# NIRVANALAN/CVPR23-E3DGE

Measured on AMD Instinct MI355X. Metric: rendered_rays_per_sec_64x64x24, higher is better.
Workload: dtype f32 (operands split f16 hi+lo, 3 f16 MFMA products, fp32 accumulate)

## Files before the change

cvpr23-e3dge_amd/csrc/siren16.h:

```cpp
#pragma once
#include "siren_common.h"

namespace e3dge {

typedef float f32x4v __attribute__((ext_vector_type(4)));

constexpr int k16Threads = 512;
constexpr int k16Tiles = 16;
constexpr int k16Steps = 8;
constexpr int k16ChunkFloats = 16 * kWidth;
constexpr int k16Chunks = kBigLayers * k16Tiles;
#ifndef E3DGE_16_ABL
#define E3DGE_16_ABL 0
#endif
constexpr int k16NBuf = 4;
constexpr int k16Slots = 2;
#ifndef E3DGE_16_RING
#define E3DGE_16_RING 2
#endif
constexpr int k16Ring = E3DGE_16_RING;

constexpr int k16LdsW = 0;
constexpr int k16LdsFilm = k16LdsW + k16NBuf * k16ChunkFloats;
constexpr int k16LdsHead = k16LdsFilm + 9 * 2 * kWidth;
constexpr int k16LdsW0 = k16LdsHead + kHeadFloats;
constexpr int k16LdsWvt = k16LdsW0 + 3 * kWidth;
constexpr int k16LdsFeat = k16LdsWvt + 3 * kWidth;
constexpr int k16LdsPart = k16LdsFeat + kRMax * kFPitch;
constexpr int k16LdsAlpha = ((k16LdsPart + 8 * k16Slots * kWidth + 3) / 4) * 4;
constexpr int k16LdsWgt = k16LdsAlpha + kTilePts;
constexpr int k16LdsZ = k16LdsWgt + kTilePts;
constexpr int k16LdsPts = k16LdsZ + kTilePts;
constexpr int k16LdsRgb = k16LdsPts + kTilePts * 3;
constexpr int k16LdsState = k16LdsRgb + kTilePts * 3;
constexpr int k16LdsWq = ((k16LdsState + kRMax * kStateStride + 3) / 4) * 4;
constexpr int k16LdsVd = k16LdsWq + 8 * k16Slots * 16;
constexpr int k16LdsFloats = k16LdsVd + 8 * 16 * 4;
constexpr int k16LdsBytes = k16LdsFloats * 4;
static_assert(k16LdsBytes <= 160 * 1024, "LDS budget");
static_assert((k16LdsFilm % 4) == 0 && (k16LdsHead % 4) == 0 && (k16LdsW0 % 4) == 0 && (k16LdsWvt % 4) == 0, "alignment");

#ifndef E3DGE_NT_STORES
#define E3DGE_NT_STORES 1
#endif
__device__ __forceinline__ void save_st4(float* p, const f32x4v& v) {
#if E3DGE_NT_STORES
    __builtin_nontemporal_store(v, reinterpret_cast<f32x4v*>(p));
#else
    *reinterpret_cast<f32x4v*>(p) = v;
#endif
}
__device__ __forceinline__ f32x4v mfma16x16(u32x4 a, u32x4 b, f32x4v c) {
    return __builtin_amdgcn_mfma_f32_16x16x32_f16(__builtin_bit_cast(half8, a), __builtin_bit_cast(half8, b), c, 0, 0, 0);
}
__device__ __forceinline__ f32x4v zero4() { return f32x4v{0.f, 0.f, 0.f, 0.f}; }
template <int HI> __device__ __forceinline__ float fma_mix_h(unsigned p, float w, float acc) {
    float r;
    if (HI) asm("v_fma_mix_f32 %0, %1, %2, %3 op_sel:[1,0,0] op_sel_hi:[1,0,0]" : "=v"(r) : "v"(p), "v"(w), "v"(acc));
    else asm("v_fma_mix_f32 %0, %1, %2, %3 op_sel:[0,0,0] op_sel_hi:[1,0,0]" : "=v"(r) : "v"(p), "v"(w), "v"(acc));
    return r;
}
__device__ __forceinline__ float act16_get(const u32x4 (&aH)[k16Steps], const u32x4 (&aL)[k16Steps], int t, int r) {
    const int g = t >> 1, w = 2 * (t & 1) + (r >> 1);
    return (r & 1) ? f16hi(aH[g][w]) + f16hi(aL[g][w]) : f16lo(aH[g][w]) + f16lo(aL[g][w]);
}
template <int CTRL> __device__ __forceinline__ float dpp16(float x) {
    return __builtin_bit_cast(float, __builtin_amdgcn_update_dpp(0, __builtin_bit_cast(int, x), CTRL, 0xf, 0xf, true));
}
__device__ __forceinline__ float row_sum16(float x) {
    x += dpp16<0x128>(x);
    x += dpp16<0x124>(x);
    x += dpp16<0x122>(x);
    x += dpp16<0x121>(x);
    return x;
}

__device__ __forceinline__ float sum_over_q(float x) {
    const unsigned u = __builtin_bit_cast(unsigned, x);
    const auto r = __builtin_amdgcn_permlane16_swap(u, u, false, false);
    const float y = __builtin_bit_cast(float, (unsigned)r[0]) + __builtin_bit_cast(float, (unsigned)r[1]);
    const unsigned v = __builtin_bit_cast(unsigned, y);
    const auto t = __builtin_amdgcn_permlane32_swap(v, v, false, false);
    return __builtin_bit_cast(float, (unsigned)t[0]) + __builtin_bit_cast(float, (unsigned)t[1]);
}

template <int CTRL, int ROW_MASK> __device__ __forceinline__ float dpp_or(float ident, float x) {
    return __builtin_bit_cast(float, __builtin_amdgcn_update_dpp(__builtin_bit_cast(int, ident), __builtin_bit_cast(int, x), CTRL, ROW_MASK, 0xf, false));
}
__device__ __forceinline__ float wave_incl_prod(float x) {
    x = __fmul_rn(x, dpp_or<0x111, 0xf>(1.0f, x));
    x = __fmul_rn(x, dpp_or<0x112, 0xf>(1.0f, x));
    x = __fmul_rn(x, dpp_or<0x114, 0xf>(1.0f, x));
    x = __fmul_rn(x, dpp_or<0x118, 0xf>(1.0f, x));
    x = __fmul_rn(x, dpp_or<0x142, 0xa>(1.0f, x));
    x = __fmul_rn(x, dpp_or<0x143, 0xc>(1.0f, x));
    return x;
}
__device__ __forceinline__ float wave_sum_last(float x) {
    x = __fadd_rn(x, dpp_or<0x111, 0xf>(0.0f, x));
    x = __fadd_rn(x, dpp_or<0x112, 0xf>(0.0f, x));
    x = __fadd_rn(x, dpp_or<0x114, 0xf>(0.0f, x));
    x = __fadd_rn(x, dpp_or<0x118, 0xf>(0.0f, x));
    x = __fadd_rn(x, dpp_or<0x142, 0xa>(0.0f, x));
    x = __fadd_rn(x, dpp_or<0x143, 0xc>(0.0f, x));
    return __builtin_bit_cast(float, __builtin_amdgcn_readlane(__builtin_bit_cast(int, x), 63));
}

struct ChunkPipe16 {
    const char* img;
    uint32_t voff, lds_base;
    int idx, buf, use_buf, count;
    float* wbuf;
    const float* wcur;
    const float* wnxt;
    __device__ __forceinline__ void init(float* wbuf_, const float* image, int wave, int lane, int count_ = k16Chunks) {
        const int wave_u = __builtin_amdgcn_readfirstlane(wave);
        wbuf = wbuf_;
        count = count_;
        img = reinterpret_cast<const char*>(image) + wave_u * 2048;
        voff = (uint32_t)lane * 16u;
        lds_base = (uint32_t)(size_t)(__attribute__((address_space(3))) float*)wbuf_ + (uint32_t)wave_u * 2048u;
        idx = 0; buf = 0; use_buf = 0;
        wcur = wbuf_; wnxt = wbuf_ + k16ChunkFloats;
    }
    __device__ __forceinline__ void issue_chunk() {
        const char* s = img + (size_t)idx * (k16ChunkFloats * 4);
        const uint32_t d = lds_base + (uint32_t)buf * (k16ChunkFloats * 4);
        glds16_saddr<0>(s, voff, d);
        glds16_saddr<1024>(s, voff, d);
        idx = (idx + 1 == count) ? 0 : idx + 1;
        buf = (buf + 1 == k16NBuf) ? 0 : buf + 1;
    }
    __device__ __forceinline__ void prime() {
        issue_chunk(); issue_chunk(); issue_chunk();
    }
#ifdef E3DGE_PHASE_TIMING
    unsigned long long t_vm = 0, t_bar = 0;
#endif
    template <bool STRICT> __device__ __forceinline__ void sync() {
#ifdef E3DGE_PHASE_TIMING
        const unsigned long long c0 = __builtin_readcyclecounter();
#endif
        if (STRICT) asm volatile("s_waitcnt vmcnt(0)" ::: "memory");
        else asm volatile("s_waitcnt vmcnt(2)" ::: "memory");
#ifdef E3DGE_PHASE_TIMING
        const unsigned long long c1 = __builtin_readcyclecounter();
#endif
#if !(E3DGE_16_ABL & 4)
        __syncthreads();
#endif
#ifdef E3DGE_PHASE_TIMING
        t_vm += c1 - c0; t_bar += __builtin_readcyclecounter() - c1;
#endif
    }
    __device__ __forceinline__ void advance() {
        use_buf = (use_buf + 1 == k16NBuf) ? 0 : use_buf + 1;
        wcur = wnxt;
        wnxt = wbuf + ((use_buf + 1 == k16NBuf) ? 0 : use_buf + 1) * k16ChunkFloats;
    }
};

#ifdef E3DGE_16_TRACE
__device__ unsigned long long g_trace16[2][24];
#define TRACE16_STAMP(i) do { if (trace) asm volatile("s_memtime %0" : "=s"(tstamp[i])); } while (0)
#else
#define TRACE16_STAMP(i) do { } while (0)
#endif

template <bool TRANSPOSED, int RING = k16Ring, class Epi, class Hook>
__device__ __forceinline__ void tile16(ChunkPipe16& pipe, int lane, const u32x4 (&aH)[k16Steps], const u32x4 (&aL)[k16Steps],
                                       f32x4v& acc, f32x4v& accb, u32x4 (&ringH)[RING], u32x4 (&ringL)[RING], Epi&& epi,
                                       Hook&& hook, int sbuf = -1, [[maybe_unused]] int trace = 0) {
#ifdef E3DGE_16_TRACE
    unsigned long long tstamp[24];
#endif
    const u32x4* __restrict__ wp = reinterpret_cast<const u32x4*>(sbuf >= 0 ? pipe.wbuf + sbuf * k16ChunkFloats : pipe.wcur) + lane;
    const u32x4* __restrict__ wn = reinterpret_cast<const u32x4*>(sbuf >= 0 ? pipe.wbuf + ((sbuf + 1) % k16NBuf) * k16ChunkFloats : pipe.wnxt) + lane;
#pragma unroll
    for (int g = 0; g < k16Steps; ++g) {
        const int ga = g + RING - 1;
        TRACE16_STAMP(3 * g);
        ringH[ga % RING] = (ga < k16Steps) ? wp[(ga * 2 + 0) * 64] : wn[((ga - k16Steps) * 2 + 0) * 64];
        ringL[ga % RING] = (ga < k16Steps) ? wp[(ga * 2 + 1) * 64] : wn[((ga - k16Steps) * 2 + 1) * 64];
        __builtin_amdgcn_sched_barrier(0);
        const u32x4 wh = ringH[g % RING], wl = ringL[g % RING];
        f32x4v& x0 = (g & 1) ? accb : acc;
        f32x4v& x1 = (g & 1) ? acc : accb;
        if (!TRANSPOSED) {
            x0 = mfma16x16(wh, aH[g], x0);
            x1 = mfma16x16(wl, aH[g], x1);
            x0 = mfma16x16(wh, aL[g], x0);
        } else {
            x0 = mfma16x16(aH[g], wh, x0);
            x1 = mfma16x16(aH[g], wl, x1);
            x0 = mfma16x16(aL[g], wh, x0);
        }
        TRACE16_STAMP(3 * g + 1);
        if (g == 1) hook();
        epi(g);
        TRACE16_STAMP(3 * g + 2);
    }
#ifdef E3DGE_16_TRACE
    if (trace) {
        asm volatile("s_waitcnt lgkmcnt(0)" ::: "memory");
        if ((threadIdx.x & 63) == 0)
            for (int i = 0; i < 24; ++i) g_trace16[trace - 1][i] = tstamp[i];
    }
#endif
}

#ifndef E3DGE_16_HELPERS_ONLY
#ifdef E3DGE_PHASE_TIMING
#define PHASE16(i) do { if (MODE == 0 && blockIdx.x == 0 && tid == 0 && sub < 3) tstamp[sub * 6 + (i)] = __builtin_readcyclecounter(); } while (0)
#else
#define PHASE16(i) do { } while (0)
#endif

constexpr int64_t k16SlabWords = 8 * 2 * 64;

template <int MODE, bool SAVE, int CACHE = 0>
__global__ void __launch_bounds__(k16Threads) siren16_kernel(const SirenK a) {
    static_assert(CACHE == 0 || (MODE == 0 && !SAVE), "the backbone hand-over exists for inference renders only");
    extern __shared__ __attribute__((aligned(16))) float smem[];
    float* const wbuf = smem + k16LdsW;
    float* const film_s = smem + k16LdsFilm;
    float* const head_s = smem + k16LdsHead;
    float* const w0_s = smem + k16LdsW0;
    float* const wvt_s = smem + k16LdsWvt;
    float* const feat_acc = smem + k16LdsFeat;
    float* const part = smem + k16LdsPart;
    float* const alpha_s = smem + k16LdsAlpha;
    float* const wgt_s = smem + k16LdsWgt;
    float* const z_s = smem + k16LdsZ;
    float* const pts_s = smem + k16LdsPts;
    float* const rgb_s = smem + k16LdsRgb;
    float* const state = smem + k16LdsState;

    const int tid_k = threadIdx.x;
#ifdef E3DGE_PHASE_TIMING
    const unsigned long long t_entry = __builtin_readcyclecounter();
    unsigned long long t_loop0 = 0, t_loop1 = 0;
#endif
    int b, npts, n_sub;
    int pix0 = 0, nrays = 0;
    long long pt0 = 0;
    const int S = (MODE == 0) ? a.S : 1;
    if (MODE == 0) {
        b = blockIdx.x / a.tiles_per_img;
        const int tile = blockIdx.x - b * a.tiles_per_img;
        const int HW = a.H * a.Wd;
        pix0 = tile * a.R;
        nrays = min(a.R, HW - pix0);
        npts = nrays * S;
    } else {
        b = blockIdx.x / a.wgs_per_img;
        const int wg = blockIdx.x - b * a.wgs_per_img;
        pt0 = (long long)wg * a.subtiles_per_wg * kTilePts;
        const long long rem = a.n_pts - pt0;
        npts = (int)(rem < (long long)a.subtiles_per_wg * kTilePts ? rem : (long long)a.subtiles_per_wg * kTilePts);
    }
    n_sub = (npts + kTilePts - 1) / kTilePts;

    const float* __restrict__ packed = a.packed;
    const float* __restrict__ film_g = a.film + (int64_t)b * 9 * 2 * kWidth;
    ChunkPipe16 pipe;
    if (CACHE == 2) pipe.init(wbuf, packed + kOffBig16b + (int64_t)(kBigLayers - 1) * k16Tiles * k16ChunkFloats, tid_k >> 6, tid_k & 63, k16Tiles);
    else pipe.init(wbuf, packed + kOffBig16b, tid_k >> 6, tid_k & 63);
    pipe.prime();
    for (int i = tid_k; i < 9 * kWidth; i += k16Threads) {
        const int l = i >> 8, n = i & 255;
        const float gm = film_g[(l * 2 + 0) * kWidth + n], bt = film_g[(l * 2 + 1) * kWidth + n];
        film_s[(l * 2 + 0) * kWidth + n] = (l >= 1) ? gm * (1.0f / kW16Scale) : gm;
        film_s[(l * 2 + 1) * kWidth + n] = __fadd_rn(__fmul_rn(gm, packed[kOffBias + l * kWidth + n]), bt);
    }
    for (int i = tid_k; i < kHeadFloats; i += k16Threads) head_s[i] = packed[kOffWSigma + i];
    for (int i = tid_k; i < 3 * kWidth; i += k16Threads) {
        const int c = i >> 8, n = i & 255;
        const int src = ((n >> 5) * 2 + (c >> 1)) * 64 + (c & 1) * 32 + (n & 31);
        w0_s[i] = packed[kOffFirst + src];
        wvt_s[i] = packed[kOffVTail + src] * kW16Scale;
    }
    float cw[12] = {0}, focal = 1.f, nearv = 0.f, farv = 0.f;
    if (MODE == 0) {
#pragma unroll
        for (int i = 0; i < 12; ++i) cw[i] = a.c2w[b * 12 + i];
        focal = a.focal[b]; nearv = a.near[b]; farv = a.far[b];
        for (int i = tid_k; i < kRMax * kStateStride; i += k16Threads) state[i] = 0.0f;
        for (int i = tid_k; i < kRMax * kFPitch; i += k16Threads) feat_acc[i] = 0.0f;
    }
    const float* __restrict__ film = film_s;

    asm volatile("s_waitcnt vmcnt(0)" ::: "memory");
    __syncthreads();
    u32x4 ringH[k16Ring], ringL[k16Ring];
    {
        const int lane0 = tid_k & 63;
#pragma unroll
        for (int g = 0; g < k16Ring - 1; ++g) {
            ringH[g] = reinterpret_cast<const u32x4*>(pipe.wcur)[(g * 2 + 0) * 64 + lane0];
            ringL[g] = reinterpret_cast<const u32x4*>(pipe.wcur)[(g * 2 + 1) * 64 + lane0];
        }
    }

#ifdef E3DGE_16_TRACE
    auto trace_sel = [&](int L, int t) {
        const int w = __builtin_amdgcn_readfirstlane(tid_k >> 6);
        return (MODE == 0 && blockIdx.x == 7 && L == 3 && t == 6 && (w == 0 || w == 4)) ? 1 + (w >> 2) : 0;
    };
#else
    auto trace_sel = [](int, int) { return 0; };
#endif
    auto fwd_hook = [&](int younger) {
        if (SAVE) {
            switch (younger) {
                case 2: asm volatile("s_waitcnt vmcnt(2)" ::: "memory"); break;
                case 3: asm volatile("s_waitcnt vmcnt(3)" ::: "memory"); break;
                default: asm volatile("s_waitcnt vmcnt(4)" ::: "memory"); break;
            }
            asm volatile("s_waitcnt lgkmcnt(0)\n\ts_barrier" ::: "memory");
        } else {
            pipe.template sync<false>();
        }
        pipe.issue_chunk();
    };
    u32x4 inH[k16Steps], inL[k16Steps], outH[k16Steps], outL[k16Steps];
#ifdef E3DGE_PHASE_TIMING
    unsigned long long tstamp[18];
    for (int i = 0; i < 18; ++i) tstamp[i] = 0;
#endif

#ifdef E3DGE_PHASE_TIMING
    t_loop0 = __builtin_readcyclecounter();
#endif
    for (int sub = 0; sub < n_sub; ++sub) {
        int tid_o = tid_k;
        asm volatile("" : "+v"(tid_o));
        const int tid = tid_o, lane = tid & 63, wave = tid >> 6, q = lane >> 4, col = lane & 15;
        PHASE16(0);
        const int p_sub = 16 * wave + col;
        const int p = sub * kTilePts + p_sub;
        const bool valid = p < npts;
        const int pc = valid ? p : (npts - 1);
        float px = 0.f, py = 0.f, pz = 0.f, vx = 0.f, vy = 0.f, vz = 0.f, zval = 0.f, dist = 0.f;
        int ray_l = 0, s_idx = 0;
        int64_t gpt;
        if (MODE == 0) {
            ray_l = pc / S;
            s_idx = pc - ray_l * S;
            const int pix = pix0 + ray_l;
            const int iy = pix / a.Wd, ix = pix - iy * a.Wd;
            gpt = ((int64_t)b * a.H * a.Wd + pix) * S + s_idx;
            const float hres = (float)a.res * 0.5f;
            const float d0 = __fdiv_rn(((float)ix + 0.5f) - hres, focal);
            const float d1 = -__fdiv_rn(((float)iy + 0.5f) - hres, focal);
            const float d2 = -1.0f;
            float rd[3];
#pragma unroll
            for (int m = 0; m < 3; ++m)
                rd[m] = __fadd_rn(__fadd_rn(__fmul_rn(d0, cw[4 * m + 0]), __fmul_rn(d1, cw[4 * m + 1])), __fmul_rn(d2, cw[4 * m + 2]));
            const float dn = sqrtf(__fadd_rn(__fadd_rn(__fmul_rn(d0, d0), __fmul_rn(d1, d1)), __fmul_rn(d2, d2)));
            vx = __fdiv_rn(d0, dn); vy = __fdiv_rn(d1, dn); vz = __fdiv_rn(d2, dn);
            const float tv = a.t_vals[s_idx];
            zval = __fadd_rn(__fmul_rn(nearv, __fsub_rn(1.0f, tv)), __fmul_rn(farv, tv));
            px = __fadd_rn(cw[3], __fmul_rn(rd[0], zval));
            py = __fadd_rn(cw[7], __fmul_rn(rd[1], zval));
            pz = __fadd_rn(cw[11], __fmul_rn(rd[2], zval));
            const float rdn = sqrtf(__fadd_rn(__fadd_rn(__fmul_rn(rd[0], rd[0]), __fmul_rn(rd[1], rd[1])), __fmul_rn(rd[2], rd[2])));
            if (s_idx + 1 < S) {
                const float tn = a.t_vals[s_idx + 1];
                const float zn = __fadd_rn(__fmul_rn(nearv, __fsub_rn(1.0f, tn)), __fmul_rn(farv, tn));
                dist = __fmul_rn(__fsub_rn(zn, zval), rdn);
            } else {
                dist = __fmul_rn(1e10f, rdn);
            }
            if (valid && q == 0) {
                if (a.points) { float* o = a.points + gpt * 3; o[0] = px; o[1] = py; o[2] = pz; }
                if (a.dists) a.dists[gpt] = dist;
                if (s_idx == 0) {
                    const int64_t gr = (int64_t)b * a.H * a.Wd + pix;
                    if (a.rays_d) { float* o = a.rays_d + gr * 3; o[0] = rd[0]; o[1] = rd[1]; o[2] = rd[2]; }
                    if (a.viewdirs) { float* o = a.viewdirs + gr * 3; o[0] = vx; o[1] = vy; o[2] = vz; }
                }
            }
        } else {
            gpt = (int64_t)b * a.n_pts + pt0 + pc;
            const float* pp = a.pts + gpt * 3;
            px = pp[0]; py = pp[1]; pz = pp[2];
            if (a.vdirs) { const float* vv = a.vdirs + gpt * 3; vx = vv[0]; vy = vv[1]; vz = vv[2]; }
        }
        const int64_t gpt_block = (MODE == 0) ? ((int64_t)b * a.H * a.Wd + pix0) * S : (int64_t)b * a.n_pts + pt0;
        const bool sblk = SAVE && a.save_blocked != 0;
        const int64_t img_n = (MODE == 0) ? (int64_t)a.H * a.Wd * S : (int64_t)a.n_pts;
        const int64_t srow_block = (int64_t)b * saved_rows_per_image(sblk, img_n) + ((MODE == 0) ? (int64_t)pix0 * S : pt0);
        float* const sv = SAVE ? a.save_args + saved_row_floats(sblk, srow_block + pc, q, 9) : nullptr;
        const int sv_ls = sblk ? kSlabLayerF : kWidth, sv_ts = sblk ? kSlabTileF : 16;
        float* const vd_s = smem + k16LdsVd + wave * 64;
        if (q == 0) { vd_s[col * 4 + 0] = vx; vd_s[col * 4 + 1] = vy; vd_s[col * 4 + 2] = vz; }

        if (CACHE != 2) {
            const float xs = __fmul_rn(px, a.box_scale), ys = __fmul_rn(py, a.box_scale), zs = __fmul_rn(pz, a.box_scale);
#pragma unroll
            for (int t = 0; t < k16Tiles; ++t) {
                const int o = 16 * t + 4 * q;
                const f32x4v wx = *reinterpret_cast<const f32x4v*>(w0_s + o), wy = *reinterpret_cast<const f32x4v*>(w0_s + kWidth + o),
                             wz = *reinterpret_cast<const f32x4v*>(w0_s + 2 * kWidth + o);
                const f32x4v g4 = *reinterpret_cast<const f32x4v*>(film + o), b4 = *reinterpret_cast<const f32x4v*>(film + kWidth + o);
                f32x4v arg, v;
#pragma unroll
                for (int r = 0; r < 4; ++r) {
                    const float lin = fmaf(wz[r], zs, fmaf(wy[r], ys, wx[r] * xs));
                    arg[r] = fmaf(g4[r], lin, b4[r]);
                    v[r] = sin_f32(arg[r]);
                }
                if (SAVE) save_st4(sv + t * sv_ts, arg);
                SPLIT2_TO(v[0], v[1], inH[t >> 1][2 * (t & 1)], inL[t >> 1][2 * (t & 1)]);
                SPLIT2_TO(v[2], v[3], inH[t >> 1][2 * (t & 1) + 1], inL[t >> 1][2 * (t & 1) + 1]);
            }
        }

        PHASE16(1);
#pragma unroll 1
        for (int L = 1; L < ((CACHE == 2) ? 0 : E3DGE_SIREN_DEPTH); ++L) {
            const float* __restrict__ film_l = film + L * 2 * kWidth;
            f32x4v prev = zero4();
            auto finish = [&](int tp, const f32x4v& pv) {
                const int o = 16 * tp + 4 * q;
                const f32x4v g4 = *reinterpret_cast<const f32x4v*>(film_l + o), b4 = *reinterpret_cast<const f32x4v*>(film_l + kWidth + o);
                f32x4v arg, v;
#pragma unroll
                for (int r = 0; r < 4; ++r) { arg[r] = fmaf(g4[r], pv[r], b4[r]); v[r] = sin_f32(arg[r]); }
                if (SAVE) save_st4(sv + L * sv_ls + tp * sv_ts, arg);
                SPLIT2_TO(v[0], v[1], outH[tp >> 1][2 * (tp & 1)], outL[tp >> 1][2 * (tp & 1)]);
                SPLIT2_TO(v[2], v[3], outH[tp >> 1][2 * (tp & 1) + 1], outL[tp >> 1][2 * (tp & 1) + 1]);
            };
#pragma unroll
            for (int t = 0; t < k16Tiles; ++t) {
                f32x4v acc = zero4(), accb = zero4();
                if (t == 0) {
                    tile16<false>(pipe, lane, inH, inL, acc, accb, ringH, ringL, [](int) {}, [&]() { fwd_hook(2); }, t % k16NBuf);
                } else {
                    const int o = 16 * (t - 1) + 4 * q;
                    f32x4v g4 = zero4(), b4 = zero4(), arg4 = zero4(), kf4 = zero4(), x4 = zero4();
                    tile16<false>(pipe, lane, inH, inL, acc, accb, ringH, ringL, [&](int g) {
                        if (g == 0) {
                            g4 = *reinterpret_cast<const f32x4v*>(film_l + o);
                            b4 = *reinterpret_cast<const f32x4v*>(film_l + kWidth + o);
                        } else if (g == 1) {
#pragma unroll
                            for (int r = 0; r < 4; ++r) arg4[r] = fmaf(g4[r], prev[r], b4[r]);
#ifndef E3DGE_POLY_SINE
#pragma unroll
                            for (int r = 0; r < 4; ++r) kf4[r] = rintf(arg4[r] * 0.15915494f);
                        } else if (g == 2) {
#pragma unroll
                            for (int r = 0; r < 4; ++r) kf4[r] = fmaf(arg4[r], 6.4206382e-09f, fmaf(arg4[r], 0.15915494f, -kf4[r]));
#endif
                        } else if (g == 3) {
#pragma unroll
#ifndef E3DGE_POLY_SINE
                            for (int r = 0; r < 4; ++r) x4[r] = __builtin_amdgcn_sinf(kf4[r]);
#else
                            for (int r = 0; r < 4; ++r) x4[r] = sin_poly_f32(arg4[r]);
#endif
                            if (SAVE) save_st4(sv + L * sv_ls + (t - 1) * sv_ts, arg4);
                        } else if (g == 4) {
                            SPLIT2_TO(x4[0], x4[1], outH[(t - 1) >> 1][2 * ((t - 1) & 1)], outL[(t - 1) >> 1][2 * ((t - 1) & 1)]);
                            SPLIT2_TO(x4[2], x4[3], outH[(t - 1) >> 1][2 * ((t - 1) & 1) + 1], outL[(t - 1) >> 1][2 * ((t - 1) & 1) + 1]);
                        }
                    }, [&]() { fwd_hook(t < 2 ? 2 : (t == 2 ? 3 : 4)); }, t % k16NBuf, trace_sel(L, t));
                }
                pipe.advance();
                prev = acc + accb;
            }
            finish(k16Tiles - 1, prev);
#pragma unroll
            for (int g = 0; g < k16Steps; ++g) { inH[g] = outH[g]; inL[g] = outL[g]; }
        }

        if (CACHE != 0) {
            const int64_t rec = (((int64_t)blockIdx.x * a.bb_subs + sub) * 8 + wave) * k16SlabWords + lane;
            if (CACHE == 1) {
                u32x4* __restrict__ dst = reinterpret_cast<u32x4*>(a.bb_out) + rec;
#pragma unroll
                for (int g = 0; g < k16Steps; ++g) { dst[(g * 2 + 0) * 64] = inH[g]; dst[(g * 2 + 1) * 64] = inL[g]; }
            } else {
                const u32x4* __restrict__ src = reinterpret_cast<const u32x4*>(a.bb_in) + rec;
#pragma unroll
                for (int g = 0; g < k16Steps; ++g) { inH[g] = src[(g * 2 + 0) * 64]; inL[g] = src[(g * 2 + 1) * 64]; }
            }
        }

        PHASE16(2);
        float sdf = 0.0f;
        if (CACHE == 2) {
            if (q == 0) wgt_s[p_sub] = valid ? a.weights_in[gpt] : 0.0f;
        } else {
            float acc = 0.0f;
#pragma unroll
            for (int t = 0; t < k16Tiles; ++t) {
                const f32x4v w4 = *reinterpret_cast<const f32x4v*>(head_s + 16 * t + 4 * q);
                const int g = t >> 1, w0i = 2 * (t & 1);
                acc = fma_mix_h<0>(inH[g][w0i], w4[0], acc); acc = fma_mix_h<0>(inL[g][w0i], w4[0], acc);
                acc = fma_mix_h<1>(inH[g][w0i], w4[1], acc); acc = fma_mix_h<1>(inL[g][w0i], w4[1], acc);
                acc = fma_mix_h<0>(inH[g][w0i + 1], w4[2], acc); acc = fma_mix_h<0>(inL[g][w0i + 1], w4[2], acc);
                acc = fma_mix_h<1>(inH[g][w0i + 1], w4[3], acc); acc = fma_mix_h<1>(inL[g][w0i + 1], w4[3], acc);
            }
            sdf = sum_over_q(acc) + head_s[4 * kWidth];
        }

        if (MODE == 0 && CACHE != 2) {
            const float sg = __fdiv_rn(sigmoid_f32(__fdiv_rn(-sdf, a.sigmoid_beta)), a.sigmoid_beta);
            const float alpha = __fsub_rn(1.0f, expf(-__fmul_rn(sg, dist)));
            if (q == 0) {
                alpha_s[p_sub] = valid ? alpha : 0.0f;
                z_s[p_sub] = zval;
                pts_s[p_sub * 3 + 0] = px; pts_s[p_sub * 3 + 1] = py; pts_s[p_sub * 3 + 2] = pz;
                if (valid && a.sdf) a.sdf[gpt] = sdf;
            }
            __syncthreads();
            const int sub_lo = sub * kTilePts;
            const int sub_hi = min(sub_lo + kTilePts, npts);
            const int r_first = sub_lo / S, r_last = (sub_hi - 1) / S;
            for (int i = __builtin_amdgcn_readfirstlane(wave); i <= ((E3DGE_16_ABL & 8) ? -1 : r_last - r_first); i += 8) {
                const int rl = r_first + i;
                const int s_lo = max(0, sub_lo - rl * S), s_hi = min(S, sub_hi - rl * S);
                float* st = state + rl * kStateStride;
                float T_in = (s_lo == 0) ? 1.0f : st[0];
                float wsum = (s_lo == 0) ? 0.0f : st[1];
                float dep = 0.0f, x0 = 0.0f, x1 = 0.0f, x2 = 0.0f;
                for (int c0 = s_lo; c0 < s_hi; c0 += 64) {
                    const int s = c0 + lane;
                    const bool act = s < s_hi;
                    const int ps = rl * S + min(s, s_hi - 1) - sub_lo;
                    const float al = act ? alpha_s[ps] : 0.0f;
                    const float zz = z_s[ps], p0 = pts_s[ps * 3 + 0], p1 = pts_s[ps * 3 + 1], p2 = pts_s[ps * 3 + 2];
                    const float incl = wave_incl_prod(act ? __fadd_rn(__fsub_rn(1.0f, al), 1e-10f) : 1.0f);
                    const float T = __fmul_rn(T_in, dpp_or<0x138, 0xf>(1.0f, incl));
                    float w = __fmul_rn(al, T);
                    const bool last = a.force_bg && act && s == S - 1;
                    const float wfront = wave_sum_last(last ? 0.0f : w);
                    if (last) w = __fsub_rn(1.0f, __fadd_rn(wsum, wfront));
                    wsum = __fadd_rn(wsum, wfront);
                    if (act) wgt_s[ps] = w;
                    dep = __fadd_rn(dep, wave_sum_last(__fmul_rn(w, zz)));
                    x0 = __fadd_rn(x0, wave_sum_last(__fmul_rn(w, p0)));
                    x1 = __fadd_rn(x1, wave_sum_last(__fmul_rn(w, p1)));
                    x2 = __fadd_rn(x2, wave_sum_last(__fmul_rn(w, p2)));
                    T_in = __fmul_rn(T_in, __builtin_bit_cast(float, __builtin_amdgcn_readlane(__builtin_bit_cast(int, incl), 63)));
                }
                if (lane == 0) {
                    st[0] = T_in; st[1] = wsum;
                    st[2] = __fadd_rn(st[2], dep); st[3] = __fadd_rn(st[3], x0); st[4] = __fadd_rn(st[4], x1); st[5] = __fadd_rn(st[5], x2);
                }
            }
            __syncthreads();
            if (valid && q == 0 && a.weights) a.weights[gpt] = wgt_s[p_sub];
        }

        if (MODE == 0 && a.tex_alpha) {
            const float* __restrict__ ta = a.tex_alpha + gpt * kWidth;
            const float* __restrict__ tb = a.tex_beta + gpt * kWidth;
#pragma unroll
            for (int t = 0; t < k16Tiles; ++t) {
                const f32x4v a4 = *reinterpret_cast<const f32x4v*>(ta + 16 * t + 4 * q);
                const f32x4v b4 = *reinterpret_cast<const f32x4v*>(tb + 16 * t + 4 * q);
                float y[4];
#pragma unroll
                for (int r = 0; r < 4; ++r) y[r] = __fadd_rn(__fmul_rn(__fadd_rn(a4[r], 1.0f), act16_get(inH, inL, t, r)), b4[r]);
                SPLIT2_TO(y[0], y[1], inH[t >> 1][2 * (t & 1)], inL[t >> 1][2 * (t & 1)]);
                SPLIT2_TO(y[2], y[3], inH[t >> 1][2 * (t & 1) + 1], inL[t >> 1][2 * (t & 1) + 1]);
            }
        }

        PHASE16(3);
        float* const wq_s = smem + k16LdsWq + wave * (k16Slots * 16);
        int slab_first_ray = 0, slab_nslots = 0;
        const int slab_p0 = sub * kTilePts + 16 * wave;
        if (MODE == 0) {
            const int slab_hi = min(slab_p0 + 16, npts);
            if (slab_hi > slab_p0) {
                slab_first_ray = slab_p0 / S;
                slab_nslots = (slab_hi - 1) / S - slab_first_ray + 1;
            }
            const int b1 = (slab_first_ray + 1) * S - slab_p0;
            if (lane < 16) {
                const float w = (slab_p0 + lane < npts) ? wgt_s[16 * wave + lane] : 0.0f;
                wq_s[lane] = (lane < b1) ? w : 0.0f;
                wq_s[16 + lane] = (lane >= b1) ? w : 0.0f;
            }
        }
        const f32x4v q0 = (MODE == 0) ? *reinterpret_cast<const f32x4v*>(wq_s + 4 * q) : zero4();
        const f32x4v q1 = (MODE == 0) ? *reinterpret_cast<const f32x4v*>(wq_s + 16 + 4 * q) : zero4();
        float dvx[4], dvy[4], dvz[4];
#pragma unroll
        for (int r = 0; r < 4; ++r) { dvx[r] = vd_s[(4 * q + r) * 4 + 0]; dvy[r] = vd_s[(4 * q + r) * 4 + 1]; dvz[r] = vd_s[(4 * q + r) * 4 + 2]; }
        float prgb[3][4];
#pragma unroll
        for (int c = 0; c < 3; ++c)
#pragma unroll
            for (int r = 0; r < 4; ++r) prgb[c][r] = 0.0f;
        {
            const float* __restrict__ film_v = film + 8 * 2 * kWidth;
            const float* __restrict__ wrgb = head_s + kWidth;
            f32x4v pv = zero4();
            float e_gm = 0.f, e_bt = 0.f, e_w0 = 0.f, e_w1 = 0.f, e_w2 = 0.f, fa0 = 0.f, fa1 = 0.f;
            int e_n = 0;
            auto epi_begin = [&](int tp) {
                e_n = 16 * tp + col;
                e_gm = film_v[e_n]; e_bt = film_v[kWidth + e_n];
                e_w0 = wrgb[e_n]; e_w1 = wrgb[kWidth + e_n]; e_w2 = wrgb[2 * kWidth + e_n];
                fa0 = fa1 = 0.f;
            };
            auto epi_r = [&](int r) {
                const float varg = fmaf(e_gm, pv[r], e_bt);
                const float h = sin_f32(varg);
                const int pr = slab_p0 + 4 * q + r;
                if (SAVE && pr < npts) a.save_args[saved_elem_floats(sblk, srow_block + pr, 8, e_n, 9)] = varg;
                prgb[0][r] = fmaf(e_w0, h, prgb[0][r]);
                prgb[1][r] = fmaf(e_w1, h, prgb[1][r]);
                prgb[2][r] = fmaf(e_w2, h, prgb[2][r]);
                if (MODE == 0) {
                    fa0 = fmaf(q0[r], h, fa0);
                    fa1 = fmaf(q1[r], h, fa1);
                } else if (a.raw) {
                    if (pr < npts) a.raw[((int64_t)b * a.n_pts + pt0 + pr) * 260 + 4 + e_n] = h;
                }
            };
            auto epi_end = [&]() {
                if (MODE == 0) {
                    fa0 = sum_over_q(fa0);
                    fa1 = sum_over_q(fa1);
                    if (q == 0) {
                        float* pp = part + (wave * k16Slots) * kWidth + e_n;
                        if (slab_nslots > 0) pp[0] = fa0;
                        if (slab_nslots > 1) pp[kWidth] = fa1;
                    }
                }
            };
#pragma unroll 1
            for (int t = 0; t < k16Tiles; ++t) {
                f32x4v acc = zero4(), accb = zero4();
                if (t == 0) {
                    tile16<true>(pipe, lane, inH, inL, acc, accb, ringH, ringL, [](int) {}, [&]() { fwd_hook(2); });
                } else {
                    epi_begin(t - 1);
                    tile16<true>(pipe, lane, inH, inL, acc, accb, ringH, ringL, [&](int g) { if (g >= 1 && g <= 4) epi_r(g - 1); }, [&]() { fwd_hook(2); });
                    epi_end();
                }
                pipe.advance();
                acc = acc + accb;
                const int n = 16 * t + col;
                const float t0 = wvt_s[n], t1 = wvt_s[kWidth + n], t2 = wvt_s[2 * kWidth + n];
#pragma unroll
                for (int r = 0; r < 4; ++r) acc[r] = fmaf(t2, dvz[r], fmaf(t1, dvy[r], fmaf(t0, dvx[r], acc[r])));
                pv = acc;
            }
            epi_begin(k16Tiles - 1);
#pragma unroll
            for (int r = 0; r < 4; ++r) epi_r(r);
            epi_end();
        }

        PHASE16(4);
        float rgbv[3][4];
#pragma unroll
        for (int c = 0; c < 3; ++c)
#pragma unroll
            for (int r = 0; r < 4; ++r) rgbv[c][r] = row_sum16(prgb[c][r]) + head_s[4 * kWidth + 1 + c];
        if (MODE == 0) {
            if (col == 0) {
#pragma unroll
                for (int r = 0; r < 4; ++r) {
                    const int ps = 16 * wave + 4 * q + r;
                    rgb_s[ps * 3 + 0] = sigmoid_f32(rgbv[0][r]);
                    rgb_s[ps * 3 + 1] = sigmoid_f32(rgbv[1][r]);
                    rgb_s[ps * 3 + 2] = sigmoid_f32(rgbv[2][r]);
                }
            }
            __syncthreads();
            const int sub_lo = sub * kTilePts;
            const int sub_hi = min(sub_lo + kTilePts, npts);
            const int r_first = sub_lo / S, r_last = (sub_hi - 1) / S;
            for (int i = __builtin_amdgcn_readfirstlane(wave); i <= ((E3DGE_16_ABL & 16) ? -1 : r_last - r_first); i += 8) {
                const int rl = r_first + i;
                const int s_lo = max(0, sub_lo - rl * S), s_hi = min(S, sub_hi - rl * S);
                float c0 = 0.0f, c1 = 0.0f, c2 = 0.0f;
                for (int b0 = s_lo; b0 < s_hi; b0 += 64) {
                    const int s = b0 + lane;
                    const int ps = rl * S + min(s, s_hi - 1) - sub_lo;
                    const float ww = (s < s_hi) ? wgt_s[ps] : 0.0f;
                    c0 = __fadd_rn(c0, wave_sum_last(__fmul_rn(ww, rgb_s[ps * 3 + 0])));
                    c1 = __fadd_rn(c1, wave_sum_last(__fmul_rn(ww, rgb_s[ps * 3 + 1])));
                    c2 = __fadd_rn(c2, wave_sum_last(__fmul_rn(ww, rgb_s[ps * 3 + 2])));
                }
                if (lane == 0) {
                    float* st = state + rl * kStateStride;
                    st[6] = __fadd_rn(st[6], c0); st[7] = __fadd_rn(st[7], c1); st[8] = __fadd_rn(st[8], c2);
                }
            }
            if (tid < kWidth && !(E3DGE_16_ABL & 32)) {
                const int n = tid;
                float pv[8 * k16Slots];
#pragma unroll
                for (int j = 0; j < 8 * k16Slots; ++j) pv[j] = part[j * kWidth + n];
                int cur = -1;
                float run = 0.0f;
#pragma unroll
                for (int wv = 0; wv < 8; ++wv) {
                    const int slab_lo = sub_lo + 16 * wv;
                    const int slab_hi2 = min(slab_lo + 16, npts);
                    if (slab_hi2 > slab_lo) {
                        const int fr = slab_lo / S;
                        const int ns = (slab_hi2 - 1) / S - fr + 1;
#pragma unroll
                        for (int sl = 0; sl < k16Slots; ++sl)
                            if (sl < ns) {
                                if (fr + sl != cur) {
                                    if (cur >= 0) feat_acc[cur * kFPitch + n] += run;
                                    cur = fr + sl;
                                    run = 0.0f;
                                }
                                run += pv[wv * k16Slots + sl];
                            }
                    }
                }
                if (cur >= 0) feat_acc[cur * kFPitch + n] += run;
            }
            __syncthreads();
        } else {
            if (a.raw && col == 0) {
#pragma unroll
                for (int r = 0; r < 4; ++r) {
                    const int pr = sub * kTilePts + 16 * wave + 4 * q + r;
                    if (pr < npts) {
                        float* o = a.raw + ((int64_t)b * a.n_pts + pt0 + pr) * 260;
                        o[0] = rgbv[0][r]; o[1] = rgbv[1][r]; o[2] = rgbv[2][r];
                    }
                }
            }
            if (valid && q == 0) {
                if (a.sdf) a.sdf[gpt] = sdf;
                if (a.raw) a.raw[gpt * 260 + 3] = sdf;
            }
        }
        PHASE16(5);
    }

#ifdef E3DGE_PHASE_TIMING
    t_loop1 = __builtin_readcyclecounter();
#endif
    asm volatile("s_waitcnt vmcnt(0)" ::: "memory");
    if (MODE == 0) {
        const int tid = tid_k;
        const int HW = a.H * a.Wd;
        if (a.features) {
            float* fo = a.features + (int64_t)b * kWidth * HW + pix0;
            for (int e = tid; e < nrays * kWidth; e += k16Threads) {
                const int n = e / nrays, rl = e - n * nrays;
                fo[(int64_t)n * HW + rl] = feat_acc[rl * kFPitch + n];
            }
        }
        for (int rl = tid; rl < nrays; rl += k16Threads) {
            const float* st = state + rl * kStateStride;
            const int pix = pix0 + rl;
            if (a.rgb) {
                float* o = a.rgb + (int64_t)b * 3 * HW + pix;
                o[0] = __fadd_rn(-1.0f, __fmul_rn(2.0f, st[6]));
                o[HW] = __fadd_rn(-1.0f, __fmul_rn(2.0f, st[7]));
                o[2 * HW] = __fadd_rn(-1.0f, __fmul_rn(2.0f, st[8]));
            }
            if (a.xyz) {
                float* o = a.xyz + (int64_t)b * 3 * HW + pix;
                o[0] = st[3]; o[HW] = st[4]; o[2 * HW] = st[5];
            }
            if (a.depth) a.depth[(int64_t)b * HW + pix] = st[2];
            if (a.mask) a.mask[(int64_t)b * HW + pix] = (st[2] < a.mask_thresh) ? 1.0f : 0.0f;
        }
#ifdef E3DGE_PHASE_TIMING
        __syncthreads();
        float* const td = a.dists ? a.dists : a.rgb;
        if (blockIdx.x == 0 && tid == 0 && td) {
            for (int i = 0; i < 18; ++i)
                td[i] = (i % 6 == 0) ? (float)(i / 6 ? tstamp[i] - tstamp[i - 1] : 0) : (float)(tstamp[i] - tstamp[i - 1]);
            td[18] = (float)pipe.t_vm; td[19] = (float)pipe.t_bar;
            td[20] = (float)(t_loop0 - t_entry);
            td[21] = (float)(t_loop1 - t_loop0);
            td[22] = (float)(__builtin_readcyclecounter() - t_loop1);
        }
#endif
    }
    asm volatile("s_waitcnt vmcnt(0)" ::: "memory");
}

__global__ void __launch_bounds__(64)
selftest_mfma16x16_kernel(float* __restrict__ cmat, const float* __restrict__ amat, const float* __restrict__ bmat, int k) {
    const int lane = threadIdx.x, q = lane >> 4, n = lane & 15;
    f32x4v acc = zero4();
    for (int kb = 0; kb < k; kb += 32) {
        u32x4 a4, b4, dummy;
#pragma unroll
        for (int w = 0; w < 4; ++w) {
            SPLIT2_TO(amat[n * k + kb + 8 * q + 2 * w], amat[n * k + kb + 8 * q + 2 * w + 1], a4[w], dummy[w]);
            SPLIT2_TO(bmat[n * k + kb + 8 * q + 2 * w], bmat[n * k + kb + 8 * q + 2 * w + 1], b4[w], dummy[w]);
        }
        acc = mfma16x16(a4, b4, acc);
    }
#pragma unroll
    for (int r = 0; r < 4; ++r) cmat[(4 * q + r) * 16 + n] = acc[r];
}

#endif

}
```

Measured before the change: 13.52 million.

## Pack view-layer epilogue constants into vec4 LDS records and software-pipeline epilogue stages

Interleaves the view layer's per-tile epilogue with the next tile's MFMA groups in six stages: the view-tail FMA, the FiLM affine, range-reduced hardware sine, RGB accumulation, feature partials and the cross-quad reduction. It does this instead of doing the dir-tail FMA and a full per-row epilogue serially. The epilogue constants (FiLM gamma/beta, the rgb weights and the view-tail weights) are repacked into two float4 records per column, so each tile needs two vector LDS loads instead of eight scalar ones. Setup global loads are batched into registers before any LDS stores to overlap their latency. The inference path also fully unrolls the tile loop with static buffer indices, which raises code size and register pressure.

```diff
diff --git a/cvpr23-e3dge_amd/csrc/siren16.h b/cvpr23-e3dge_amd/csrc/siren16.h
--- a/cvpr23-e3dge_amd/csrc/siren16.h
+++ b/cvpr23-e3dge_amd/csrc/siren16.h
@@ -24,8 +24,8 @@
 constexpr int k16LdsFilm = k16LdsW + k16NBuf * k16ChunkFloats;
 constexpr int k16LdsHead = k16LdsFilm + 9 * 2 * kWidth;
 constexpr int k16LdsW0 = k16LdsHead + kHeadFloats;
-constexpr int k16LdsWvt = k16LdsW0 + 3 * kWidth;
-constexpr int k16LdsFeat = k16LdsWvt + 3 * kWidth;
+constexpr int k16LdsVrec = k16LdsW0 + 3 * kWidth;
+constexpr int k16LdsFeat = k16LdsVrec + 2 * 4 * kWidth;
 constexpr int k16LdsPart = k16LdsFeat + kRMax * kFPitch;
 constexpr int k16LdsAlpha = ((k16LdsPart + 8 * k16Slots * kWidth + 3) / 4) * 4;
 constexpr int k16LdsWgt = k16LdsAlpha + kTilePts;
@@ -38,7 +38,7 @@
 constexpr int k16LdsFloats = k16LdsVd + 8 * 16 * 4;
 constexpr int k16LdsBytes = k16LdsFloats * 4;
 static_assert(k16LdsBytes <= 160 * 1024, "LDS budget");
-static_assert((k16LdsFilm % 4) == 0 && (k16LdsHead % 4) == 0 && (k16LdsW0 % 4) == 0 && (k16LdsWvt % 4) == 0, "alignment");
+static_assert((k16LdsFilm % 4) == 0 && (k16LdsHead % 4) == 0 && (k16LdsW0 % 4) == 0 && (k16LdsVrec % 4) == 0, "alignment");
 
 #ifndef E3DGE_NT_STORES
 #define E3DGE_NT_STORES 1
@@ -226,7 +226,7 @@
     float* const film_s = smem + k16LdsFilm;
     float* const head_s = smem + k16LdsHead;
     float* const w0_s = smem + k16LdsW0;
-    float* const wvt_s = smem + k16LdsWvt;
+    float* const vrec_s = smem + k16LdsVrec;
     float* const feat_acc = smem + k16LdsFeat;
     float* const part = smem + k16LdsPart;
     float* const alpha_s = smem + k16LdsAlpha;
@@ -267,18 +267,60 @@
     if (CACHE == 2) pipe.init(wbuf, packed + kOffBig16b + (int64_t)(kBigLayers - 1) * k16Tiles * k16ChunkFloats, tid_k >> 6, tid_k & 63, k16Tiles);
     else pipe.init(wbuf, packed + kOffBig16b, tid_k >> 6, tid_k & 63);
     pipe.prime();
-    for (int i = tid_k; i < 9 * kWidth; i += k16Threads) {
-        const int l = i >> 8, n = i & 255;
-        const float gm = film_g[(l * 2 + 0) * kWidth + n], bt = film_g[(l * 2 + 1) * kWidth + n];
-        film_s[(l * 2 + 0) * kWidth + n] = (l >= 1) ? gm * (1.0f / kW16Scale) : gm;
-        film_s[(l * 2 + 1) * kWidth + n] = __fadd_rn(__fmul_rn(gm, packed[kOffBias + l * kWidth + n]), bt);
-    }
-    for (int i = tid_k; i < kHeadFloats; i += k16Threads) head_s[i] = packed[kOffWSigma + i];
-    for (int i = tid_k; i < 3 * kWidth; i += k16Threads) {
-        const int c = i >> 8, n = i & 255;
+    constexpr int kFilmIt = (9 * kWidth + k16Threads - 1) / k16Threads;
+    constexpr int kHeadIt = (kHeadFloats + k16Threads - 1) / k16Threads;
+    constexpr int kColIt = (3 * kWidth + k16Threads - 1) / k16Threads;
+    float ld_gm[kFilmIt], ld_bt[kFilmIt], ld_bias[kFilmIt], ld_head[kHeadIt], ld_w0[kColIt], ld_vt[kColIt];
+#pragma unroll
+    for (int j = 0; j < kFilmIt; ++j) {
+        const int i = tid_k + j * k16Threads, l = i >> 8, n = i & 255;
+        ld_gm[j] = ld_bt[j] = ld_bias[j] = 0.0f;
+        if (i < 9 * kWidth) {
+            ld_gm[j] = film_g[(l * 2 + 0) * kWidth + n];
+            ld_bt[j] = film_g[(l * 2 + 1) * kWidth + n];
+            ld_bias[j] = packed[kOffBias + l * kWidth + n];
+        }
+    }
+#pragma unroll
+    for (int j = 0; j < kHeadIt; ++j) {
+        const int i = tid_k + j * k16Threads;
+        ld_head[j] = (i < kHeadFloats) ? packed[kOffWSigma + i] : 0.0f;
+    }
+#pragma unroll
+    for (int j = 0; j < kColIt; ++j) {
+        const int i = tid_k + j * k16Threads, c = i >> 8, n = i & 255;
         const int src = ((n >> 5) * 2 + (c >> 1)) * 64 + (c & 1) * 32 + (n & 31);
-        w0_s[i] = packed[kOffFirst + src];
-        wvt_s[i] = packed[kOffVTail + src] * kW16Scale;
+        ld_w0[j] = ld_vt[j] = 0.0f;
+        if (i < 3 * kWidth) { ld_w0[j] = packed[kOffFirst + src]; ld_vt[j] = packed[kOffVTail + src]; }
+    }
+#pragma unroll
+    for (int j = 0; j < kFilmIt; ++j) {
+        const int i = tid_k + j * k16Threads, l = i >> 8, n = i & 255;
+        if (i < 9 * kWidth) {
+            const float gm = ld_gm[j], bt = ld_bt[j];
+            const float g_s = (l >= 1) ? gm * (1.0f / kW16Scale) : gm;
+            const float b_s = __fadd_rn(__fmul_rn(gm, ld_bias[j]), bt);
+            film_s[(l * 2 + 0) * kWidth + n] = g_s;
+            film_s[(l * 2 + 1) * kWidth + n] = b_s;
+            if (l == 8) { vrec_s[4 * n + 0] = g_s; vrec_s[4 * n + 1] = b_s; }
+        }
+    }
+#pragma unroll
+    for (int j = 0; j < kHeadIt; ++j) {
+        const int i = tid_k + j * k16Threads;
+        if (i < kHeadFloats) {
+            head_s[i] = ld_head[j];
+            const int c = (i >> 8) - 1, n = i & 255;
+            if (c >= 0 && c < 3) vrec_s[(c == 2 ? 4 * kWidth : 0) + 4 * n + (c == 2 ? 0 : 2 + c)] = ld_head[j];
+        }
+    }
+#pragma unroll
+    for (int j = 0; j < kColIt; ++j) {
+        const int i = tid_k + j * k16Threads, c = i >> 8, n = i & 255;
+        if (i < 3 * kWidth) {
+            w0_s[i] = ld_w0[j];
+            vrec_s[4 * kWidth + 4 * n + 1 + c] = ld_vt[j] * kW16Scale;
+        }
     }
     float cw[12] = {0}, focal = 1.f, nearv = 0.f, farv = 0.f;
     if (MODE == 0) {
@@ -600,65 +642,82 @@
 #pragma unroll
             for (int r = 0; r < 4; ++r) prgb[c][r] = 0.0f;
         {
-            const float* __restrict__ film_v = film + 8 * 2 * kWidth;
-            const float* __restrict__ wrgb = head_s + kWidth;
-            f32x4v pv = zero4();
-            float e_gm = 0.f, e_bt = 0.f, e_w0 = 0.f, e_w1 = 0.f, e_w2 = 0.f, fa0 = 0.f, fa1 = 0.f;
-            int e_n = 0;
-            auto epi_begin = [&](int tp) {
-                e_n = 16 * tp + col;
-                e_gm = film_v[e_n]; e_bt = film_v[kWidth + e_n];
-                e_w0 = wrgb[e_n]; e_w1 = wrgb[kWidth + e_n]; e_w2 = wrgb[2 * kWidth + e_n];
-                fa0 = fa1 = 0.f;
+            const f32x4v* __restrict__ vra = reinterpret_cast<const f32x4v*>(vrec_s) + col;
+            const f32x4v* __restrict__ vrb = reinterpret_cast<const f32x4v*>(vrec_s + 4 * kWidth) + col;
+            f32x4v ra = zero4(), rb = zero4(), pacc = zero4(), paccb = zero4(), pv = zero4(), varg = zero4(), kf = zero4(), hv = zero4();
+            float fa0 = 0.f, fa1 = 0.f;
+            auto epi = [&](int tp, int g) {
+                const int e_n = 16 * tp + col;
+                if (g == 0) {
+                    const f32x4v s4 = pacc + paccb;
+#pragma unroll
+                    for (int r = 0; r < 4; ++r) pv[r] = fmaf(rb[3], dvz[r], fmaf(rb[2], dvy[r], fmaf(rb[1], dvx[r], s4[r])));
+                } else if (g == 1) {
+#pragma unroll
+                    for (int r = 0; r < 4; ++r) varg[r] = fmaf(ra[0], pv[r], ra[1]);
+#ifndef E3DGE_POLY_SINE
+#pragma unroll
+                    for (int r = 0; r < 4; ++r) kf[r] = rintf(varg[r] * 0.15915494f);
+                } else if (g == 2) {
+#pragma unroll
+                    for (int r = 0; r < 4; ++r) kf[r] = fmaf(varg[r], 6.4206382e-09f, fmaf(varg[r], 0.15915494f, -kf[r]));
+#pragma unroll
+                    for (int r = 0; r < 4; ++r) hv[r] = __builtin_amdgcn_sinf(kf[r]);
+#else
+                } else if (g == 2) {
+#pragma unroll
+                    for (int r = 0; r < 4; ++r) hv[r] = sin_poly_f32(varg[r]);
+#endif
+                } else if (g == 3) {
+#pragma unroll
+                    for (int r = 0; r < 4; ++r) {
+                        const int pr = slab_p0 + 4 * q + r;
+                        if (SAVE && pr < npts) a.save_args[saved_elem_floats(sblk, srow_block + pr, 8, e_n, 9)] = varg[r];
+                        if (MODE != 0 && a.raw && pr < npts) a.raw[((int64_t)b * a.n_pts + pt0 + pr) * 260 + 4 + e_n] = hv[r];
+                    }
+#pragma unroll
+                    for (int r = 0; r < 4; ++r) {
+                        prgb[0][r] = fmaf(ra[2], hv[r], prgb[0][r]);
+                        prgb[1][r] = fmaf(ra[3], hv[r], prgb[1][r]);
+                        prgb[2][r] = fmaf(rb[0], hv[r], prgb[2][r]);
+                    }
+                } else if (g == 4) {
+                    if (MODE == 0) {
+                        fa0 = fa1 = 0.f;
+#pragma unroll
+                        for (int r = 0; r < 4; ++r) { fa0 = fmaf(q0[r], hv[r], fa0); fa1 = fmaf(q1[r], hv[r], fa1); }
+                    }
+                } else if (g == 5) {
+                    if (MODE == 0) {
+                        fa0 = sum_over_q(fa0);
+                        fa1 = sum_over_q(fa1);
+                        if (q == 0) {
+                            float* pp = part + (wave * k16Slots) * kWidth + e_n;
+                            if (slab_nslots > 0) pp[0] = fa0;
+                            if (slab_nslots > 1) pp[kWidth] = fa1;
+                        }
+                    }
+                }
             };
-            auto epi_r = [&](int r) {
-                const float varg = fmaf(e_gm, pv[r], e_bt);
-                const float h = sin_f32(varg);
-                const int pr = slab_p0 + 4 * q + r;
-                if (SAVE && pr < npts) a.save_args[saved_elem_floats(sblk, srow_block + pr, 8, e_n, 9)] = varg;
-                prgb[0][r] = fmaf(e_w0, h, prgb[0][r]);
-                prgb[1][r] = fmaf(e_w1, h, prgb[1][r]);
-                prgb[2][r] = fmaf(e_w2, h, prgb[2][r]);
-                if (MODE == 0) {
-                    fa0 = fmaf(q0[r], h, fa0);
-                    fa1 = fmaf(q1[r], h, fa1);
-                } else if (a.raw) {
-                    if (pr < npts) a.raw[((int64_t)b * a.n_pts + pt0 + pr) * 260 + 4 + e_n] = h;
-                }
+            auto load_rec = [&](int t) { ra = vra[16 * t]; rb = vrb[16 * t]; };
+            auto view_tile = [&](int t, int sbuf) {
+                f32x4v acc = zero4(), accb = zero4();
+                tile16<true>(pipe, lane, inH, inL, acc, accb, ringH, ringL, [&](int g) {
+                    if (t > 0 && g <= 5) epi(t - 1, g);
+                    if (g == 4) load_rec(t);
+                }, [&]() { fwd_hook(2); }, sbuf);
+                pipe.advance();
+                pacc = acc; paccb = accb;
             };
-            auto epi_end = [&]() {
-                if (MODE == 0) {
-                    fa0 = sum_over_q(fa0);
-                    fa1 = sum_over_q(fa1);
-                    if (q == 0) {
-                        float* pp = part + (wave * k16Slots) * kWidth + e_n;
-                        if (slab_nslots > 0) pp[0] = fa0;
-                        if (slab_nslots > 1) pp[kWidth] = fa1;
-                    }
-                }
-            };
+            if constexpr (MODE == 0 && !SAVE) {
+#pragma unroll
+                for (int t = 0; t < k16Tiles; ++t) view_tile(t, t % k16NBuf);
+            } else {
 #pragma unroll 1
-            for (int t = 0; t < k16Tiles; ++t) {
-                f32x4v acc = zero4(), accb = zero4();
-                if (t == 0) {
-                    tile16<true>(pipe, lane, inH, inL, acc, accb, ringH, ringL, [](int) {}, [&]() { fwd_hook(2); });
-                } else {
-                    epi_begin(t - 1);
-                    tile16<true>(pipe, lane, inH, inL, acc, accb, ringH, ringL, [&](int g) { if (g >= 1 && g <= 4) epi_r(g - 1); }, [&]() { fwd_hook(2); });
-                    epi_end();
-                }
-                pipe.advance();
-                acc = acc + accb;
-                const int n = 16 * t + col;
-                const float t0 = wvt_s[n], t1 = wvt_s[kWidth + n], t2 = wvt_s[2 * kWidth + n];
-#pragma unroll
-                for (int r = 0; r < 4; ++r) acc[r] = fmaf(t2, dvz[r], fmaf(t1, dvy[r], fmaf(t0, dvx[r], acc[r])));
-                pv = acc;
-            }
-            epi_begin(k16Tiles - 1);
-#pragma unroll
-            for (int r = 0; r < 4; ++r) epi_r(r);
-            epi_end();
+                for (int t = 0; t < k16Tiles; ++t) view_tile(t, -1);
+            }
+#pragma unroll
+            for (int g = 0; g <= 5; ++g) epi(k16Tiles - 1, g);
         }
 
         PHASE16(4);
```

Result: faster. 13.87 million, median of 6 (+2.6%).
